# Spimp/sparc_ldpc

Measured on AMD Instinct MI355X. Metric: decoded codewords/sec (T AMP iters) at L=512,M=512; achieved HBM GB/s vs roofline, higher is better.
Workload: dtype f32; 1 GPU; BASELINE configs[1]: L=512 M=512 R=1 P=4, T=64, single codeword; L=512, M=512, n=4608, T=64, backend=hadamard, precision=fp32, early_stop=False, parallelism=reps sharded over 1 GPU(s)

## Files before the change

### include/sparc_amp.h

```cpp
#ifndef SPARC_AMP_H
#define SPARC_AMP_H

#include <stdint.h>

#ifdef __cplusplus
extern "C" {
#endif

typedef struct sa_ctx sa_ctx;

enum {
  SA_OK = 0,
  SA_ERR_ARG = -1,
  SA_ERR_HIP = -2,
  SA_ERR_NOMEM = -3,
  SA_ERR_ORDERING = -4,
  SA_ERR_UNSUPPORTED = -5,
  SA_ERR_NO_DEVICE = -6
};

enum {
  SA_BACKEND_HADAMARD = 0,
  SA_BACKEND_DENSE = 1,
  SA_BACKEND_HOST = 2,
// ... 17 lines not shown
  SA_PLAN_NO_SEC3 = 1 << 1,
  SA_PLAN_ROW16 = 1 << 2,
  SA_PLAN_NO_ROW16 = 1 << 3,
  SA_PLAN_NO_PT = 1 << 4,
  SA_PLAN_ZIL = 1 << 5,
  SA_PLAN_NO_ZIL = 1 << 6,
  SA_PLAN_WB8 = 1 << 7,
  SA_PLAN_WB16 = 1 << 8,
  SA_PLAN_NO_BANKS = 1 << 9,
  SA_PLAN_EAGER = 1 << 10,
  SA_PLAN_ONE_PASS = 1 << 11,
  SA_PLAN_NO_LANES = 1 << 12,
  SA_PLAN_SEC4Q = 1 << 13,
  SA_PLAN_NO_SEC4Q = 1 << 14,
  SA_PLAN_NO_FUSED_TAIL = 1 << 15,
  SA_PLAN_ALL = (1 << 16) - 1
};
int sa_create_ex(sa_ctx** out, int L, int M, int n, const uint32_t* ordering,
                 int backend, int precision, int device, int plan);

int sa_create_matrix(sa_ctx** out, int L, int M, int n, const double* A,
                     int precision, int device);

int sa_create_matrix_random(sa_ctx** out, int L, int M, int n, uint64_t seed, double scale,
                            int precision, int device);

int sa_subset(const sa_ctx* parent, const int64_t* sections, int Ls, sa_ctx** out);

int sa_create_twin(sa_ctx* src, sa_ctx** out);

void sa_destroy(sa_ctx* ctx);
// ... 108 lines not shown
```

### sparc_ldpc_amd/_lib.py

```python
from __future__ import annotations

import ctypes as ct
import os

import numpy as np

LIB_NAME = "libsparc_amp.so"
LIB_PATH = os.environ.get("SPARC_AMP_LIB") or os.path.join(os.path.dirname(os.path.abspath(__file__)), LIB_NAME)

SA_OK = 0
SA_ERR_ARG = -1
SA_ERR_HIP = -2
SA_ERR_NOMEM = -3
SA_ERR_ORDERING = -4
SA_ERR_UNSUPPORTED = -5
SA_ERR_NO_DEVICE = -6

SA_BACKEND_HADAMARD = 0
SA_BACKEND_DENSE = 1
SA_BACKEND_HOST = 2
SA_BACKEND_MATRIX = 3
SA_PREC_F32 = 0
SA_PREC_F64 = 1
SA_FLAG_NO_EARLY_STOP = 1
SA_FLAG_BETA0 = 0x100
SA_PTR_DEVICE = 0x200
SA_SE_MAX_M = 4096
SA_LLR_MODES = {"reference": 0, "two_sided": 1}

SA_PLAN = {
    "SEC3": 1 << 0, "NO_SEC3": 1 << 1, "ROW16": 1 << 2, "NO_ROW16": 1 << 3, "NO_PT": 1 << 4,
    "ZIL": 1 << 5, "NO_ZIL": 1 << 6, "WB8": 1 << 7, "WB16": 1 << 8, "NO_BANKS": 1 << 9, "EAGER": 1 << 10,
    "ONE_PASS": 1 << 11, "NO_LANES": 1 << 12, "SEC4Q": 1 << 13, "NO_SEC4Q": 1 << 14,
    "NO_FUSED_TAIL": 1 << 15,
}


def plan_bits(plan) -> int:
    if plan is None:
        return 0
    if isinstance(plan, int):
        return plan
    if isinstance(plan, str):
        plan = [plan]
    bits = 0
    for name in plan:
        key = name.upper()
        if key not in SA_PLAN:
            raise ValueError(f"unknown plan option {name!r}; known: {sorted(SA_PLAN)}")
# ... 142 lines not shown
```

### sparc_ldpc_amd/csrc/sa_common.h

```cpp
#pragma once
#include <hip/hip_runtime.h>
#include <hip/hip_ext.h>

#include <cfloat>
#include <cmath>
#include <cstdint>
#include <cstdio>
#include <cstdlib>
#include <cstring>
#include <algorithm>
#include <map>
#include <random>
#include <thread>
#include <string>
#include <tuple>
#include <type_traits>
#include <vector>

#include "sparc_amp.h"
#include "sa_shape.h"

namespace sa {

extern thread_local std::string g_err;
// ... 702 lines not shown
enum { SEC_AMP = 0, SEC_AZ = 1, SEC_AB = 2 };
enum { ROW_INIT0 = 0, ROW_INIT = 1, ROW_AMP = 2, ROW_ABOUT = 3 };


template <typename real>
struct SecArgs {
  const uint16_t* __restrict__ inv;
  const uint16_t* __restrict__ invb;
  const uint16_t* __restrict__ invl;
  const uint32_t* __restrict__ hs;
  const ushort4* __restrict__ fwd;
  const ushort4* __restrict__ fwdb;
  const uint32_t* __restrict__ fwd2;
  const uint32_t* __restrict__ fwd3;
  const uint32_t* __restrict__ inv32;
  const real* __restrict__ c;
  const real* __restrict__ z;
  real* __restrict__ beta;
  real* __restrict__ beta_out;
  real* __restrict__ out;
  real* __restrict__ abp;
  real* __restrict__ bbp;
  const real* __restrict__ zzp;
  real* __restrict__ tau;
  int* __restrict__ iters;
  int L, M, n, w, nhi, G, NZ, T1, t, mode, early_stop;
  int cst;
  int RS;
  int pt;
  int B, NC;
  int zil;
  int gpx;
  real sqrt_n;
  const int* tb;
  int dead;
  int bzero;
  int32_t* dec;
  int itset;
};

template <typename real>
struct RowArgs {
  const real* __restrict__ tau;
  const real* __restrict__ y;
  const real* __restrict__ z_in;
  const real* __restrict__ bbp;
  const real* __restrict__ Pb;
  const real* __restrict__ abp;
  int n, G, Gb, NZ, T1, t, mode, early_stop;
  int Pbst;
  int pt;
  int Bc;
  int itset;
// ... 91 lines not shown
      int e0 = elem_index<E>(lane, i);
      e0 = e0 < M ? e0 : 0;
      const unsigned bo = (off0 + (unsigned)(h * M + e0)) * 2u;
      if constexpr (Q == 4) {
        tb[hh][i / Q] = ld_off(reinterpret_cast<const ushort4*>(base), bo);
      } else if constexpr (Q == 2) {
        const ushort2 t2 = ld_off(reinterpret_cast<const ushort2*>(base), bo);
        tb[hh][i / Q] = make_ushort4(t2.x, t2.y, 0, 0);
      } else {
        tb[hh][i / Q] = make_ushort4(ld_off(base, bo), 0, 0, 0);
      }
    }
  }
}

template <typename real, int E, int KH>
__device__ __forceinline__ void gather_buckets(const real* zs, int h0, int nhi,
                                               const ushort4 (&tb)[KH][(E + 3) / 4], real (&v)[E]) {
  constexpr int Q = E < 4 ? E : 4;
  if constexpr (KH * E <= 64) {
    if (h0 + KH <= nhi) {
      real zz[KH][E];
#pragma unroll
      for (int hh = 0; hh < KH; ++hh)
#pragma unroll
        for (int i = 0; i < E; i += Q) {
          const ushort4 r4 = tb[hh][i / Q];
          const unsigned short rr[4] = {r4.x, r4.y, r4.z, r4.w};
#pragma unroll
          for (int q = 0; q < Q; ++q) {
// ... 92 lines not shown
```

### sparc_ldpc_amd/csrc/sa_host.h

```cpp
#pragma once
#include "sa_common.h"
#include "sa_tables.h"

namespace sa {

struct Prof {
  std::vector<std::tuple<int, hipEvent_t, hipEvent_t>> ev;
  int rep = 1;
  bool dispatch = false;
  int kind = 0;
  int begin(hipStream_t s, int k) {
    kind = k;
    if (dispatch) return 0;
    hipEvent_t a = nullptr, b = nullptr;
    if (add(&a, &b)) return -1;
    return hipEventRecord(a, s) == hipSuccess ? 0 : -1;
  }
  void end(hipStream_t s) {
    if (!dispatch) (void)hipEventRecord(std::get<2>(ev.back()), s);
  }
  int add(hipEvent_t* a, hipEvent_t* b) {
    *a = *b = nullptr;
    if (hipEventCreate(a) != hipSuccess || hipEventCreate(b) != hipSuccess) return -1;
    ev.emplace_back(kind, *a, *b);
// ... 144 lines not shown
  a.abp = (real*)ln.d_abp; a.bbp = (real*)ln.d_bbp; a.zzp = (const real*)ln.d_zzp;
  a.tau = (real*)ln.d_tau; a.iters = ln.d_iters;
  a.L = c->L; a.M = c->M; a.n = c->n; a.w = c->w; a.nhi = c->nhi; a.G = c->G; a.NZ = p.nz;
  a.T1 = c->Tcap + 1; a.t = t; a.mode = mode; a.early_stop = early_stop;
  a.RS = 1;
  a.pt = 0;
  a.B = 0; a.NC = 0; a.zil = 0; a.gpx = 1 << 20;
  a.cst = c->pb_on ? c->L : 0;
  if (c->pb_on) a.c = (const real*)c->d_cb;
  a.sqrt_n = (real)std::sqrt((double)c->n);
  a.tb = tb;
  a.dead = c->dead;
  a.bzero = 0;
  a.dec = nullptr;
  a.itset = 0;
  return a;
}

template <typename real>
RowArgs<real> row_args(sa_ctx* c, const Plan& p, int mode, int t, int early_stop, int G, int Gb, const int* tb = nullptr) {
  RowArgs<real> a;
  const sa_lane& ln = c->at();
  a.y = (const real*)ln.d_y; a.z = (real*)ln.d_z; a.z_in = a.z; a.abp = (const real*)ln.d_abp;
  a.bbp = (const real*)ln.d_bbp; a.zzp = (real*)ln.d_zzp; a.tau = (const real*)ln.d_tau;
  a.out = (real*)c->d_out;
  a.n = c->n; a.G = G; a.NZ = p.nz;
  a.Gb = Gb; a.T1 = c->Tcap + 1; a.t = t; a.mode = mode;
  a.early_stop = early_stop;
  a.sqrt_n = c->backend != SA_BACKEND_HADAMARD ? (real)1 : (real)std::sqrt((double)c->n);
  a.Pb = c->pb_on ? (const real*)c->d_Pb : (const real*)c->d_P1;
// ... 105 lines not shown
```

### sparc_ldpc_amd/csrc/sa_host_check.cpp

```cpp
#include <algorithm>
#include <cstdio>
#include <cstdlib>
#include <cstring>
#include <numeric>

#include "sa_shape.h"
#include "sa_tables.h"

using namespace sa;

static int usage() {
  std::fprintf(stderr, "usage: sa_host_check shape L M n backend prec plan n_cus B\n"
                       "       sa_host_check sweep L M backend prec plan n_cus B n0 n1\n"
                       "       sa_host_check tables L M n prec plan\n");
  return 2;
}

static int shape_of(Shape& s, int L, int M, int n, int backend, int prec, int plan, int n_cus) {
  std::string err;
  int rc = SA_OK;
  if (L <= 0 || M <= 0 || n <= 0 || n_cus <= 0 || backend < SA_BACKEND_HADAMARD || backend > SA_BACKEND_MATRIX ||
      (prec != SA_PREC_F32 && prec != SA_PREC_F64) || (plan & ~SA_PLAN_ALL)) {
    rc = SA_ERR_ARG;
    err = "bad arguments";
  }
  if (!rc) rc = shape_limits(M, n, backend, err);
  if (!rc) rc = shape_for(s, L, M, n, backend, prec, plan, n_cus, err);
  if (rc) std::printf("{\"error\": %d, \"message\": \"%s\"}\n", rc, err.c_str());
  return rc;
// ... 212 lines not shown
  std::vector<uint16_t> inv, fwd;
  std::vector<uint32_t> inv32;
  if (s.big ? check_inv(s, ord, inv32) : check_inv(s, ord, inv)) return 1;
  if (check_fwd(s, ord, fwd)) return 1;
  const bool secb = s.CB > 0 && !s.big, banked = invb_banked(s);
  if (secb && check_fwdb(s, fwd)) return 1;
  if (banked && check_banked(s, inv)) return 1;
  std::printf("{\"ok\": 1, \"M\": %d, \"dead\": %d, \"w\": %d, \"E\": %d, \"big\": %d, \"sec3\": %d, \"CB\": %d, \"WB\": %d, "
              "\"fwdb\": %d, \"fwdb_lanes\": %d, \"banked\": %d, \"kh\": %d, \"search\": %d}\n",
              s.M, s.dead, s.w, s.E, s.big ? 1 : 0, s.sec3 ? 1 : 0, s.CB, s.WB, secb ? 1 : 0,
              secb ? (s.CB * (int)rsz(&s) == 16 ? 16 : 32) : 0, banked ? 1 : 0, banked ? invb_kh(s) : 0,
              (plan & SA_PLAN_NO_BANKS) ? 0 : 1);
  return 0;
}

int main(int argc, char** argv) {
  if (argc < 2) return usage();
  std::vector<int> a;
  for (int i = 2; i < argc; ++i) a.push_back(std::atoi(argv[i]));
  if (!std::strcmp(argv[1], "shape") && a.size() == 8) return cmd_shape(a[0], a[1], a[2], a[3], a[4], a[5], a[6], a[7]);
  if (!std::strcmp(argv[1], "sweep") && a.size() == 9)
    return cmd_sweep(a[0], a[1], a[2], a[3], a[4], a[5], a[6], a[7], a[8]);
  if (!std::strcmp(argv[1], "tables") && a.size() == 5) return cmd_tables(a[0], a[1], a[2], a[3], a[4]);
  return usage();
}
```

### sparc_ldpc_amd/csrc/sa_sec.hip

```cpp
#include "sa_host.h"

namespace sa {



template <typename real, int E>
__global__ void __launch_bounds__(256) k_sec(SecArgs<real> a) {
  STAMP(0);
  extern __shared__ __attribute__((aligned(16))) unsigned char smem[];
  constexpr int KH = E >= 16 ? 2 : (E >= 8 ? 16 : 16);
  constexpr int NQ = (E + 3) / 4;
  constexpr int KR = 8;
  int g, rsi;
  if (a.RS > 1 && (a.G & 7) == 0) {
    const int j = blockIdx.x, u = j >> 3;
    rsi = u % a.RS;
    g = (u / a.RS) * 8 + (j & 7);
  } else {
    g = blockIdx.x / a.RS;
    rsi = blockIdx.x % a.RS;
  }
  const int b = blockIdx.y;
  const int rows_per = (a.n + a.RS - 1) / a.RS;
  const int rb0 = rsi * rows_per, rb1 = min(a.n, rb0 + rows_per);
// ... 466 lines not shown
template <typename real, int QW, bool MAX>
__device__ __forceinline__ real combine_q(const real* red, int w0, int f) {
  real x[QW];
#pragma unroll
  for (int j = 0; j < QW; ++j) x[j] = red[(w0 + j) * 4 + f];
#pragma unroll
  for (int span = 1; span < QW; span <<= 1)
#pragma unroll
    for (int j = 0; j < QW; j += 2 * span) {
      if constexpr (MAX) x[j] = x[j] > x[j + span] ? x[j] : x[j + span];
      else x[j] = x[j] + x[j + span];
    }
  return x[0];
}

template <typename real, int EQ, int QW, int SPW = 2>
__device__ __forceinline__ void secq_body(const SecArgs<real>& a) {
  static_assert(SPW == 2 || SPW == 3 || SPW == 4, "sections per workgroup");
  STAMP(0);
  extern __shared__ __attribute__((aligned(16))) unsigned char smem[];
  constexpr int NT = SPW * QW * 64;
  constexpr int KH = EQ >= 8 ? 4 : ((SPW == 3 || (SPW == 4 && sizeof(real) == 8)) ? 8 : 16);
  constexpr int NQ = (EQ + 3) / 4;
  constexpr int KR = ((SPW == 3 ? 8448 : 4608) + NT - 1) / NT;
  constexpr int FW = SPW == 4 ? 2 : 1;
  const int g = blockIdx.x, b = blockIdx.y;
  const int tid = threadIdx.x, lane = tid & 63, wv = tid >> 6;
  const int sidx = wv / QW, q = wv % QW;
  const int M = a.M, n = a.n, Mq = M / QW;
  const size_t LM = (size_t)a.L * M;
  const int l = g * SPW + sidx;
  const bool have = l < a.L;
  const int lc = have ? l : a.L - 1;
// ... 3 lines not shown
  const int zslots = ((n + 1) * (int)sizeof(real) + 15) / 16 * 16 / (int)sizeof(real);
  real* ts = zs + zslots;
  real* xb = ts + SPW * M;
  real* red = xb + SPW * M;

  real v[EQ];
  real bprev[EQ];
  const real* bl = a.beta + (size_t)b * LM + (size_t)lc * M + eoff;
  real* blo = a.beta_out + (size_t)b * LM + (size_t)lc * M + eoff;
  const uint16_t* ibase = a.inv + (size_t)g * SPW * a.w;
  const unsigned ioff = (unsigned)((lc - g * SPW) * a.w + eoff);
  const uint32_t* fw = (SPW == 3 ? a.fwd3 : a.fwd2) + (size_t)(SPW == 4 ? 2 * g : g) * n;
  const uint32_t* fw1 = a.fwd2 + (size_t)(2 * g + 1 < (a.L + 1) / 2 ? 2 * g + 1 : 2 * g) * n;
  ushort4 tb[KH][NQ];
  uint32_t f[KR][FW];

  const real* zb = a.z + (size_t)b * n;
  ZStage<real, NT> zst;
  const real* zzb = a.zzp + (size_t)b * a.NZ;
  ZZParts<real, 5> zz;
  const bool dma = stage_z_dma<real, NT>(zb, zs, n, tid);
  if (!dma) zst.issue(zb, n, tid);
  zz.issue(zzb, a.NZ, lane);
  const real last = a.t > 0 ? ld_vmem(a.tau + (size_t)b * a.T1 + a.t - 1) : (real)0;
  load_buckets_off<EQ, KH>(ibase, ioff, 0, a.nhi, M, lane, tb);
  load_section<real, EQ>(bl, bprev, lane, Mq);
  const real cl = ld_vmem(a.c + (size_t)b * a.cst + lc);
  const real tau = zz.tau(zzb, a.NZ, n);
  if (a.bzero) {
#pragma unroll
    for (int i = 0; i < EQ; ++i) bprev[i] = 0;
  }
  const bool stop = a.early_stop && (tau == last);
  if (g == 0 && tid == 0) {
    a.tau[(size_t)b * a.T1 + a.t] = tau;
    if (stop && a.iters[b] < 0) a.iters[b] = a.t;
    if (a.itset != 0 && !stop) a.iters[b] = a.itset;
  }
  if (stop) {
    if (dma) asm volatile("s_waitcnt vmcnt(0)" ::: "memory");
    if (a.bzero && have) {
      store_section<real, EQ>(a.beta + (size_t)b * LM + (size_t)lc * M + eoff, bprev, lane, Mq);
// ... 3 lines not shown
  const real tau2 = tau * tau;
  const real inv_sn = (real)1 / a.sqrt_n;
  const real kk = cl / tau2;
  STAMP(1);
  if (!dma) zst.store(zs, zb, n, tid);
  else finish_z_dma<real>(zb, zs, n, tid);
  __syncthreads();
  STAMP(2);
#ifdef SA_STAMPS
  asm volatile("s_waitcnt vmcnt(0)" ::: "memory");
  STAMP(10);
#endif
#pragma unroll
  for (int i = 0; i < EQ; ++i) v[i] = 0;
  for (int h0 = 0; h0 < a.nhi; h0 += KH) {
    ushort4 tn[KH][NQ];
    const bool more = h0 + KH < a.nhi;
    if (more) load_buckets_off<EQ, KH>(ibase, ioff, h0 + KH, a.nhi, M, lane, tn);
    gather_buckets<real, EQ, KH>(zs, h0, a.nhi, tb, v);
    if (more) {
#pragma unroll
      for (int hh = 0; hh < KH; ++hh)
#pragma unroll
        for (int j = 0; j < NQ; ++j) tb[hh][j] = tn[hh][j];
    }
  }
  real* xs = xb + sidx * M;
#pragma unroll
  for (int u = 0; u < KR; ++u) {
    const int r = u * NT + tid;
    f[u][0] = ld_off(fw, (unsigned)(r < n ? r : 0) * 4u);
    if constexpr (SPW == 4) f[u][1] = ld_off(fw1, (unsigned)(r < n ? r : 0) * 4u);
  }
  STAMP(3);
  fwht_wave<real, EQ>(v, lane, 64);
  topq_stage<real, EQ, QW>(v, xs, lane, q);
  STAMP(4);


  real mx = neg_inf<real>();
#pragma unroll
  for (int i = 0; i < EQ; ++i) {
    v[i] = fma(v[i], inv_sn, bprev[i]) * kk;
    mx = v[i] > mx ? v[i] : mx;
  }
  mx = wave_max(mx);
  if (lane == 0) red[wv * 4] = mx;
// ... 32 lines not shown
    for (int m = 32; m >= 1; m >>= 1) {
      const real ob = __shfl_xor(dbest, m);
      const int oi = __shfl_xor(dbi, m);
      if (ob > dbest || (ob == dbest && oi < dbi)) { dbest = ob; dbi = oi; }
    }
  }

  STAMP(5);
  fwht_wave<real, EQ>(v, lane, 64);
  topq_stage<real, EQ, QW>(v, xs, lane, q);
  STAMP(6);
  {
    real* tl = ts + sidx * M + eoff;
#pragma unroll
    for (int i = 0; i < EQ; ++i) tl[elem_index<EQ>(lane, i)] = v[i];
  }
  if (lane == 0) {
    red[wv * 4 + 3] = bb;
    if (a.dec) {
      red[wv * 4] = dbest;
      red[wv * 4 + 1] = (real)dbi;
    }
  }
  __syncthreads();
  STAMP(7);
  if (a.dec && have && q == 0 && lane == 0) {
    real best = red[wv * 4];
    int bi = (int)red[wv * 4 + 1];
#pragma unroll
    for (int j = 1; j < QW; ++j) {
// ... 9 lines not shown
    if constexpr (SPW == 4) bsum += red[3 * QW * 4 + 3];
    a.bbp[(size_t)b * a.G + g] = bsum;
  }
  real* abp = a.abp + ((size_t)b * a.G + g) * n;
  const int psh = a.pt == 16 ? 4 : 5;
  const size_t npad = (size_t)((n + (1 << psh) - 1) >> psh) << psh;
  real* abq = a.abp + (size_t)b * a.G * npad + ((size_t)g << psh);
  real* const sbase = a.pt ? abq : abp;
  const int sh = a.pt ? psh : 31;
  const size_t gstride = (size_t)a.G << sh;
  const int smask = (int)((1u << sh) - 1u);
  static_assert(NT % 32 == 0, "a pass of rows is a whole number of row blocks");
  const size_t ustep = sh < 31 ? (size_t)(NT >> sh) * gstride : (size_t)NT;
  for (int r0 = 0; r0 < n; r0 += NT * KR) {
    if (r0 > 0) {
#pragma unroll
      for (int u = 0; u < KR; ++u) {
        const int r = r0 + u * NT + tid;
        f[u][0] = fw[r < n ? r : 0];
        if constexpr (SPW == 4) f[u][1] = fw1[r < n ? r : 0];
      }
    }
    real* const pbase = sbase + (size_t)((r0 + tid) >> sh) * gstride + ((r0 + tid) & smask);
    auto row = [&](int u, int r) {
      real t;
      if constexpr (SPW == 2) {
        const uint32_t e = f[u][0];
        const real v0 = ts[e & 0x7fffu];
        const real v1 = ts[M + ((e >> 16) & 0x7fffu)];
        t = (e & 0x8000u) ? -v0 : v0;
        t += (e & 0x80000000u) ? -v1 : v1;
      } else if constexpr (SPW == 4) {
        const uint32_t e = f[u][0], e1 = f[u][1];
        const real v0 = ts[e & 0x7fffu];
        const real v1 = ts[M + ((e >> 16) & 0x7fffu)];
        const real v2 = ts[2 * M + (e1 & 0x7fffu)];
        const real v3 = ts[3 * M + ((e1 >> 16) & 0x7fffu)];
        t = (e & 0x8000u) ? -v0 : v0;
        t += (e & 0x80000000u) ? -v1 : v1;
        real t1 = (e1 & 0x8000u) ? -v2 : v2;
        t1 += (e1 & 0x80000000u) ? -v3 : v3;
// ... 21 lines not shown
#pragma unroll
      for (int u = 0; u < KR; ++u) {
        const int r = r0 + u * NT + tid;
        if (r < n) row(u, r);
      }
    }
  }
#ifdef SA_STAMPS
  STAMP(8);
  asm volatile("s_waitcnt vmcnt(0)" ::: "memory");
  STAMP(9);
#endif
}

template <typename real, int E4>
__global__ void __launch_bounds__(512) k_sec4(SecArgs<real> a) { secq_body<real, E4, 4, 2>(a); }
template <typename real, int E4>
__global__ void __launch_bounds__(768) k_sec43(SecArgs<real> a) { secq_body<real, E4, 4, 3>(a); }
template <typename real, int E4>
__global__ void __launch_bounds__(1024) k_sec44(SecArgs<real> a) { secq_body<real, E4, 4, 4>(a); }

template <typename real, int E>
void launch_sec_e(sa_ctx* c, const Plan& p, int B, SecArgs<real> a) {
  a.RS = p.rs;
  dim3 grid(c->G * a.RS, B);
  if (c->prof) c->prof->begin(c->at().stream, K_SEC);
  if (c->big)
    plaunch(c, k_secg<real, E>, grid, 256, c->sec_lds, a);
  else
    plaunch(c, k_sec<real, E>, grid, 256, c->sec_lds, a);
  if (c->prof) c->prof->end(c->at().stream);
}

template <typename real>
int launch_sec2(sa_ctx* c, const Plan& p, int B, int t, int es, void* bin, void* bout, int bzero, int32_t* dec,
                int itset) {
  SecArgs<real> a = sec_args<real>(c, p, SEC_AMP, t, es);
  a.pt = p.pt;
  if (bzero && !p.bzero()) return fail(SA_ERR_UNSUPPORTED, "k_sec2 reads its previous estimate");
  if ((dec || itset) && (!p.bzero() || es || c->dead))
    return fail(SA_ERR_UNSUPPORTED, "launch_sec2: no fused decision on this path");
  a.bzero = bzero;
  a.dec = dec;
  a.itset = itset;
  a.beta = (real*)bin;
  a.beta_out = (real*)bout;
  a.G = p.G;
  dim3 grid(a.G, B);
  if (c->prof) c->prof->begin(c->at().stream, K_SEC);
  switch (p.sec) {
    case SA_SEC_K_SEC43:
      switch (c->M / 256) {
        case 1: plaunch(c, k_sec43<real, 1>, grid, 768, c->sec3_lds, a); break;
        case 2: plaunch(c, k_sec43<real, 2>, grid, 768, c->sec3_lds, a); break;
        default: return fail(SA_ERR_UNSUPPORTED, "k_sec43: M");
      }
      break;
    case SA_SEC_K_SEC44:
      switch (c->M / 256) {
        case 1: plaunch(c, k_sec44<real, 1>, grid, 1024, c->sec4q_lds, a); break;
        case 2: plaunch(c, k_sec44<real, 2>, grid, 1024, c->sec4q_lds, a); break;
        default: return fail(SA_ERR_UNSUPPORTED, "k_sec44: M");
// ... 89 lines not shown
```

### sparc_ldpc_amd/csrc/sa_shape.h

```cpp
#pragma once
#include <algorithm>
#include <cstddef>
#include <string>

#include "sparc_amp.h"

namespace sa {

constexpr int kSpw = 4;
constexpr int kRowsPerBlk = 64;
constexpr int kRow2Rows = 32;
constexpr int kSG = 16;
constexpr size_t kSecbL2 = (size_t)5 << 19;
constexpr int kWB = 8, kWB16 = 16;
constexpr int kInvbZeroRows = 16;
constexpr int kSecbKH32 = 2, kSecbKH64 = 2;
constexpr size_t kLdsBytes = 160 * 1024;

inline int ilog2(int x) {
  int r = 0;
  while ((1 << r) < x) ++r;
  return r;
}

struct Shape {
  int L = 0, n = 0, backend = 0, prec = 0;
  int plan = 0;
  int n_cus = 256;
  int M = 0, Mu = 0, dead = 0;
  bool pow2 = true;
  int w = 0, nhi = 0, E = 1;
  bool big = false;
  int NZ = 0, NZ16 = 0, NZh = 0, NZ4 = 0, NZ2 = 0;
  bool row16 = false;
  bool pt_on = false;
  int G = 0;
  size_t sec_lds = 0;
  int G2 = 0;
  size_t sec2_lds = 0;
  bool sec4 = false;
  size_t sec4_lds = 0;
  int G3 = 0;
  bool sec3 = false;
  size_t sec3_lds = 0;
  int G4 = 0;
  bool sec4q = false;
  size_t sec4q_lds = 0;
  int WB = 8;
  int CB = 0;
  int Gb = 0;
  int gpx = 1 << 20;
  size_t secb_lds = 0;
  int Gd = 0;
};

inline size_t rsz(const Shape* s) { return s->prec == SA_PREC_F64 ? 8 : 4; }

inline size_t zbytes(int n, size_t s) { return ((size_t)(n + 1) * s + 15) / 16 * 16; }
inline size_t sec_lds_need(int M, int n, size_t s, bool z) {
  return (z ? zbytes(n, s) : 0) + (size_t)kSpw * M * s + (size_t)kSpw * s;
}
inline size_t sec2_need(int M, int n, size_t s) {
// ... 99 lines not shown
    const bool over = c.G2 > c.n_cus || (s == 8 && c.G2 == c.n_cus);
    const bool want = (plan & SA_PLAN_SEC3) ? true : (plan & SA_PLAN_NO_SEC3) ? false : (over && G3 <= c.n_cus);
    if (fits && want) {
      c.sec3 = true;
      c.G3 = G3;
      c.sec3_lds = sec43_need(M, n, s);
    }
    const bool fits4q = c.sec4 && backend == SA_BACKEND_HADAMARD && M <= 512 && sec44_need(M, n, s) <= kLdsBytes;
    if (fits4q && (plan & SA_PLAN_SEC4Q) && !(plan & (SA_PLAN_SEC3 | SA_PLAN_NO_SEC4Q))) {
      c.sec4q = true;
      c.sec3 = false;
      c.G4 = (L + 3) / 4;
      c.sec4q_lds = sec44_need(M, n, s);
    }
    if (c.G2 == c.n_cus && !(plan & (SA_PLAN_ROW16 | SA_PLAN_NO_SEC3))) c.row16 = false;
  }
  return SA_OK;
}

constexpr int kI8MinB = 4;
constexpr int kI8MaxS = 16;
constexpr int kFMinB = 4;
constexpr int kFMaxS = 16;

inline bool is_dense(const Shape& c) { return c.backend == SA_BACKEND_DENSE || c.backend == SA_BACKEND_MATRIX; }
inline bool use_i8(const Shape& c, int B) { return c.backend == SA_BACKEND_DENSE && B >= kI8MinB; }
inline bool use_fgemm(const Shape& c, int B) { return c.backend == SA_BACKEND_MATRIX && B >= kFMinB; }
inline bool use_batched(const Shape& c, int B) { return c.CB > 0 && B >= 4; }

inline bool zil_for(const Shape& c, int B) {
// ... 78 lines not shown
```

### sparc_ldpc_amd/csrc/sa_tables.h

```cpp
#pragma once
#include <cstdint>
#include <random>
#include <vector>

#include "sa_shape.h"

namespace sa {

struct Tables {
  uint16_t* inv = nullptr;
  uint32_t* inv32 = nullptr;
  uint16_t* invb = nullptr;
  uint16_t* invl = nullptr;
  uint32_t* hs = nullptr;
  uint16_t* fwd = nullptr;
  uint16_t* fwdb = nullptr;
  uint32_t* fwd2 = nullptr;
  uint32_t* fwd3 = nullptr;
  bool invb_done = false;
};

inline uint16_t fwd_entry(uint32_t v, int lgM, int M) {
  return (uint16_t)((v & (uint32_t)(M - 1)) | ((__builtin_popcount(v >> lgM) & 1u) << 15));
}

inline int fwd_groups(int L) { return (L + kSG - 1) / kSG * (kSG / kSpw); }

template <typename T>
bool inv_row(const uint32_t* o, int l, int n, int w, T* il, std::string& bad) {
  for (int r = 0; r < n; ++r) {
    const uint32_t v = o[r];
    if (v == 0 || v >= (uint32_t)w) {
      bad = "ordering[" + std::to_string(l) + "," + std::to_string(r) + "] = " + std::to_string(v) +
// ... 6 lines not shown
    }
    il[v] = (T)r;
  }
  return true;
}

inline void fwd_section(const uint32_t* o, int l, int n, int M, uint16_t* fwd, uint32_t* fwd2, uint32_t* fwd3) {
  const int lgM = ilog2(M);
  for (int r = 0; r < n; ++r) {
    const uint16_t e = fwd_entry(o[r], lgM, M);
    fwd[((size_t)(l / kSpw) * n + r) * kSpw + (l % kSpw)] = e;
    if (fwd2) fwd2[(size_t)(l / 2) * n + r] |= (uint32_t)e << (16 * (l & 1));
    if (fwd3)
      fwd3[(size_t)(l / 3) * n + r] |= (uint32_t)((e & 0x1ffu) | ((e >> 15) << 9)) << (10 * (l % 3));
  }
}

constexpr int kLdsGroups16[4][16] = {
    {0, 1, 2, 3, 12, 13, 14, 15, 20, 21, 22, 23, 24, 25, 26, 27},
    {4, 5, 6, 7, 8, 9, 10, 11, 16, 17, 18, 19, 28, 29, 30, 31},
    {32, 33, 34, 35, 44, 45, 46, 47, 52, 53, 54, 55, 56, 57, 58, 59},
    {36, 37, 38, 39, 40, 41, 42, 43, 48, 49, 50, 51, 60, 61, 62, 63}};

inline bool secb_rows16(const Shape& c) {
  return c.backend == SA_BACKEND_HADAMARD && c.CB > 0 && c.CB * (int)rsz(&c) == 16 && !c.big;
}
inline bool invb_banked(const Shape& c) {
  return secb_rows16(c) && !(c.plan & SA_PLAN_NO_BANKS) && c.E >= 4 && c.nhi >= 2 && c.n + kInvbZeroRows <= 65535;
}
inline int invb_kh(const Shape& c) { return c.prec == SA_PREC_F32 ? kSecbKH32 : kSecbKH64; }
// ... 196 lines not shown
```

### sparc_ldpc_amd/csrc/sa_tables.hip

```cpp

#include "sa_host.h"

namespace sa {

void tables_free(Tables& t) {
  void* all[] = {t.inv, t.inv32, t.invb, t.invl, t.hs, t.fwd, t.fwdb, t.fwd2, t.fwd3};
  for (void* p : all) dev_free(p);
  t = Tables();
}

template <typename T>
static int table_upload(sa_ctx* c, T** dst, const std::vector<T>& src) {
  if (int rc = dev_alloc(c, (void**)dst, src.size() * sizeof(T))) return rc;
  HIP_TRY(hipMemcpyAsync(*dst, src.data(), src.size() * sizeof(T), hipMemcpyHostToDevice, c->at().stream));
  return SA_OK;
}

template <typename T>
static int fill_inv(const sa_ctx* c, std::vector<T>& inv) {
  const int L = c->L, n = c->n, w = c->w;
  inv.assign((size_t)L * w, (T)n);
  std::vector<std::string> bad((size_t)L);
  parallel_for(L, 1, [&](int l) {
    inv_row(c->ordering.data() + (size_t)l * n, l, n, w, inv.data() + (size_t)l * w, bad[l]);
// ... 26 lines not shown
static void host_drop(sa_ctx* c) {
  std::vector<uint16_t>().swap(c->h_inv);
  std::vector<uint16_t>().swap(c->h_fwd);
}

int build_tables(sa_ctx* c) {
  Tables& t = c->tab;
  std::vector<uint32_t> inv32, fwd2, fwd3;
  int rc = c->big ? fill_inv(c, inv32) : fill_inv(c, c->h_inv);
  if (rc) return rc;
  fill_fwd(c, c->h_fwd, c->big ? nullptr : &fwd2, c->sec3 ? &fwd3 : nullptr);
  rc = c->big ? table_upload(c, &t.inv32, inv32) : table_upload(c, &t.inv, c->h_inv);
  if (!rc) rc = table_upload(c, &t.fwd, c->h_fwd);
  if (!rc && !c->big) rc = table_upload(c, &t.fwd2, fwd2);
  if (!rc && c->sec3) rc = table_upload(c, &t.fwd3, fwd3);
  HIP_TRY(hipStreamSynchronize(c->at().stream));
  if (rc) return rc;
  if (!(c->backend == SA_BACKEND_HADAMARD && c->CB > 0)) host_drop(c);
  return SA_OK;
}

static int build_banked(sa_ctx* c) {
  const int L = c->L, w = c->w;
  const std::vector<int> sets = invb_sets(c->E, c->prec == SA_PREC_F32);
  const uint16_t* inv = host_inv(c).data();
  std::vector<uint16_t> out((size_t)L * w, 0);
  std::vector<uint32_t> hs((size_t)L, 0);
  parallel_for(L, 1, [&](int l) {
    banked_section(c->M, c->n, c->nhi, l, inv + (size_t)l * w, out.data() + (size_t)l * w, sets, 16, 16, hs.data(),
                   invb_kh(*c));
// ... 60 lines not shown
```

Measured before the change: 2371 codewords/s.

## Bit-pack inverse bucket and forward pair tables to cut table traffic

```diff
diff --git a/include/sparc_amp.h b/include/sparc_amp.h
--- a/include/sparc_amp.h
+++ b/include/sparc_amp.h
@@ -55,7 +55,8 @@
   SA_PLAN_SEC4Q = 1 << 13,
   SA_PLAN_NO_SEC4Q = 1 << 14,
   SA_PLAN_NO_FUSED_TAIL = 1 << 15,
-  SA_PLAN_ALL = (1 << 16) - 1
+  SA_PLAN_NO_PACK = 1 << 16,
+  SA_PLAN_ALL = (1 << 17) - 1
 };
 int sa_create_ex(sa_ctx** out, int L, int M, int n, const uint32_t* ordering,
                  int backend, int precision, int device, int plan);
diff --git a/sparc_ldpc_amd/_lib.py b/sparc_ldpc_amd/_lib.py
--- a/sparc_ldpc_amd/_lib.py
+++ b/sparc_ldpc_amd/_lib.py
@@ -32,7 +32,7 @@
     "SEC3": 1 << 0, "NO_SEC3": 1 << 1, "ROW16": 1 << 2, "NO_ROW16": 1 << 3, "NO_PT": 1 << 4,
     "ZIL": 1 << 5, "NO_ZIL": 1 << 6, "WB8": 1 << 7, "WB16": 1 << 8, "NO_BANKS": 1 << 9, "EAGER": 1 << 10,
     "ONE_PASS": 1 << 11, "NO_LANES": 1 << 12, "SEC4Q": 1 << 13, "NO_SEC4Q": 1 << 14,
-    "NO_FUSED_TAIL": 1 << 15,
+    "NO_FUSED_TAIL": 1 << 15, "NO_PACK": 1 << 16,
 }
 
 
diff --git a/sparc_ldpc_amd/csrc/sa_common.h b/sparc_ldpc_amd/csrc/sa_common.h
--- a/sparc_ldpc_amd/csrc/sa_common.h
+++ b/sparc_ldpc_amd/csrc/sa_common.h
@@ -740,6 +740,8 @@
   const uint32_t* __restrict__ fwd2;
   const uint32_t* __restrict__ fwd3;
   const uint32_t* __restrict__ inv32;
+  const uint32_t* __restrict__ invp;
+  const uint64_t* __restrict__ fwd2p;
   const real* __restrict__ c;
   const real* __restrict__ z;
   real* __restrict__ beta;
@@ -763,6 +765,7 @@
   int bzero;
   int32_t* dec;
   int itset;
+  int pj;
 };
 
 template <typename real>
@@ -884,6 +887,46 @@
   }
 }
 
+using u4v = unsigned __attribute__((ext_vector_type(4)));
+
+template <int E, int KH>
+__device__ __forceinline__ void load_packed(const uint32_t* __restrict__ base, unsigned woff, int blk, int lane,
+                                            uint32_t (&pw)[pack_rd(E, KH)]) {
+  constexpr int RD = pack_rd(E, KH), NV = RD / 4;
+  const unsigned b0 = woff + (unsigned)blk * (64u * RD * 4u);
+#pragma unroll
+  for (int v = 0; v < NV; ++v) {
+    const u4v t = ld_off(reinterpret_cast<const u4v*>(base), b0 + (unsigned)(v * 256 + lane * 4) * 4u);
+    pw[4 * v] = t.x; pw[4 * v + 1] = t.y; pw[4 * v + 2] = t.z; pw[4 * v + 3] = t.w;
+  }
+#pragma unroll
+  for (int j = 4 * NV; j < RD; ++j) pw[j] = ld_off(base, b0 + (unsigned)(NV * 256 + (j - 4 * NV) * 64 + lane) * 4u);
+}
+
+template <int E, int KH>
+__device__ __forceinline__ void unpack_pairs(const uint32_t (&pw)[pack_rd(E, KH)], uint32_t (&tw)[KH]) {
+  static_assert(E <= 2, "packed records: one dword per step");
+#pragma unroll
+  for (int hh = 0; hh < KH; ++hh) {
+    uint32_t w = 0;
+#pragma unroll
+    for (int i = 0; i < E; ++i) {
+      const int bit = (hh * E + i) * kPackBits, dw = bit / 32, sh = bit % 32;
+      uint32_t x = pw[dw] >> sh;
+      if (sh + kPackBits > 32) x |= pw[dw + 1] << (32 - sh);
+      w |= (x & ((1u << kPackBits) - 1u)) << (16 * i);
+    }
+    asm("" : "+v"(w));
+    tw[hh] = w;
+  }
+}
+template <int KH>
+__device__ __forceinline__ void pairs_to_buckets(const uint32_t (&tw)[KH], ushort4 (&tb)[KH][1]) {
+#pragma unroll
+  for (int hh = 0; hh < KH; ++hh)
+    tb[hh][0] = make_ushort4((unsigned short)(tw[hh] & 0xffffu), (unsigned short)(tw[hh] >> 16), 0, 0);
+}
+
 template <typename real, int E, int KH>
 __device__ __forceinline__ void gather_buckets(const real* zs, int h0, int nhi,
                                                const ushort4 (&tb)[KH][(E + 3) / 4], real (&v)[E]) {
diff --git a/sparc_ldpc_amd/csrc/sa_host.h b/sparc_ldpc_amd/csrc/sa_host.h
--- a/sparc_ldpc_amd/csrc/sa_host.h
+++ b/sparc_ldpc_amd/csrc/sa_host.h
@@ -182,6 +182,7 @@
   a.bzero = 0;
   a.dec = nullptr;
   a.itset = 0;
+  a.invp = nullptr; a.fwd2p = nullptr; a.pj = 0;
   return a;
 }
 
diff --git a/sparc_ldpc_amd/csrc/sa_host_check.cpp b/sparc_ldpc_amd/csrc/sa_host_check.cpp
--- a/sparc_ldpc_amd/csrc/sa_host_check.cpp
+++ b/sparc_ldpc_amd/csrc/sa_host_check.cpp
@@ -12,7 +12,8 @@
 static int usage() {
   std::fprintf(stderr, "usage: sa_host_check shape L M n backend prec plan n_cus B\n"
                        "       sa_host_check sweep L M backend prec plan n_cus B n0 n1\n"
-                       "       sa_host_check tables L M n prec plan\n");
+                       "       sa_host_check tables L M n prec plan\n"
+                       "       sa_host_check packed L M n prec plan\n");
   return 2;
 }
 
@@ -255,6 +256,75 @@
   return 0;
 }
 
+static int cmd_packed(int L, int M, int n, int prec, int plan) {
+  Shape s;
+  if (shape_of(s, L, M, n, SA_BACKEND_HADAMARD, prec, plan, Shape().n_cus)) return 1;
+  size_t invp_bytes = 0, fwd2p_bytes = 0;
+  if (s.pack_inv || s.pack_fwd) {
+    std::vector<uint32_t> ord((size_t)L * n), all(s.w - 1);
+    for (int l = 0; l < L; ++l) {
+      std::mt19937 rng(0x0d0000u + (uint32_t)l);
+      std::iota(all.begin(), all.end(), 1u);
+      std::shuffle(all.begin(), all.end(), rng);
+      std::copy(all.begin(), all.begin() + n, ord.begin() + (size_t)l * n);
+    }
+    std::vector<uint16_t> inv((size_t)L * s.w, (uint16_t)n), fwd((size_t)fwd_groups(L) * n * kSpw, 0);
+    std::vector<uint32_t> fwd2((size_t)s.G2 * n, 0);
+    for (int l = 0; l < L; ++l) {
+      std::string bad;
+      CHECK(inv_row(ord.data() + (size_t)l * n, l, n, s.w, inv.data() + (size_t)l * s.w, bad), "inv_row: %s", bad.c_str());
+      fwd_section(ord.data() + (size_t)l * n, l, n, s.M, fwd.data(), fwd2.data(), nullptr);
+    }
+    if (s.pack_inv) {
+      const int kh = s.pack_kh, EQ = s.M / 256, rd = pack_rd(EQ, kh);
+      CHECK(EQ >= 1 && EQ <= 2 && n <= kPackMaxN, "packed bucket records at M = %d, n = %d", s.M, n);
+      const size_t per = pack_inv_section_dwords(s.M, s.nhi, kh);
+      CHECK(per == (size_t)4 * ((s.nhi + kh - 1) / kh) * 64 * rd, "section size");
+      std::vector<int> seen((size_t)64 * rd, 0);
+      for (int lane = 0; lane < 64; ++lane)
+        for (int j = 0; j < rd; ++j) {
+          const unsigned pos = pack_dword_pos(rd, lane, j);
+          CHECK(pos < (unsigned)(64 * rd) && !seen[pos]++, "pack_dword_pos(%d, %d, %d) = %u", rd, lane, j, pos);
+        }
+      std::vector<uint32_t> invp((size_t)L * per, 0);
+      for (int l = 0; l < L; ++l) pack_inv_section(s.M, n, s.nhi, kh, inv.data() + (size_t)l * s.w, invp.data() + (size_t)l * per);
+      for (int l = 0; l < L; ++l)
+        for (int h = 0; h < s.nhi; ++h)
+          for (int col = 0; col < s.M; ++col) {
+            const uint32_t got = pack_inv_get(s.M, s.nhi, kh, invp.data() + (size_t)l * per, h, col);
+            CHECK(got == inv[(size_t)l * s.w + (size_t)h * s.M + col], "invp[%d] step %d column %d = %u, inv has %u", l, h, col,
+                  got, (unsigned)inv[(size_t)l * s.w + (size_t)h * s.M + col]);
+          }
+      for (int l = 0; l < L; ++l)
+        for (int h = s.nhi; h < (s.nhi + kh - 1) / kh * kh; ++h)
+          for (int col = 0; col < s.M; ++col)
+            CHECK(pack_inv_get(s.M, s.nhi, kh, invp.data() + (size_t)l * per, h, col) == (uint32_t)n,
+                  "invp[%d] step %d (past nhi) column %d is not the zero slot", l, h, col);
+      invp_bytes = invp.size() * 4;
+    }
+    if (s.pack_fwd) {
+      CHECK(s.M <= 512 && !s.sec4q, "packed pair table at M = %d, quads %d", s.M, s.sec4q ? 1 : 0);
+      const int words = pack_fwd_words(n);
+      const size_t per = (size_t)words * kPackNT;
+      std::vector<uint64_t> fwd2p((size_t)s.G2 * per, 0);
+      for (int g = 0; g < s.G2; ++g) pack_fwd_pair(n, fwd2.data() + (size_t)g * n, fwd2p.data() + (size_t)g * per);
+      for (int g = 0; g < s.G2; ++g)
+        for (int r = 0; r < words * 3 * kPackNT; ++r) {
+          const uint32_t want = fwd2[(size_t)g * n + (r < n ? r : 0)], got = pack_fwd_get(fwd2p.data() + (size_t)g * per, r);
+          CHECK(got == want, "fwd2p[%d] row %d = %#x, fwd2 has %#x", g, r, got, want);
+        }
+      for (uint64_t wv : fwd2p) CHECK((wv >> 60) == 0, "fwd2p: bits past the three fields");
+      fwd2p_bytes = fwd2p.size() * 8;
+    }
+  }
+  std::printf("{\"ok\": 1, \"M\": %d, \"n\": %d, \"nhi\": %d, \"pack_inv\": %d, \"pack_fwd\": %d, \"kh\": %d, \"rd\": %d, "
+              "\"blocks\": %d, \"words\": %d, \"inv_bytes\": %zu, \"invp_bytes\": %zu, \"fwd2_bytes\": %zu, \"fwd2p_bytes\": %zu}\n",
+              s.M, n, s.nhi, s.pack_inv ? 1 : 0, s.pack_fwd ? 1 : 0, s.pack_kh,
+              s.pack_inv ? pack_rd(s.M / 256, s.pack_kh) : 0, s.pack_inv ? (s.nhi + s.pack_kh - 1) / s.pack_kh : 0,
+              s.pack_fwd ? pack_fwd_words(n) : 0, (size_t)L * s.w * 2, invp_bytes, (size_t)s.G2 * n * 4, fwd2p_bytes);
+  return 0;
+}
+
 int main(int argc, char** argv) {
   if (argc < 2) return usage();
   std::vector<int> a;
@@ -263,5 +333,6 @@
   if (!std::strcmp(argv[1], "sweep") && a.size() == 9)
     return cmd_sweep(a[0], a[1], a[2], a[3], a[4], a[5], a[6], a[7], a[8]);
   if (!std::strcmp(argv[1], "tables") && a.size() == 5) return cmd_tables(a[0], a[1], a[2], a[3], a[4]);
+  if (!std::strcmp(argv[1], "packed") && a.size() == 5) return cmd_packed(a[0], a[1], a[2], a[3], a[4]);
   return usage();
 }
diff --git a/sparc_ldpc_amd/csrc/sa_sec.hip b/sparc_ldpc_amd/csrc/sa_sec.hip
--- a/sparc_ldpc_amd/csrc/sa_sec.hip
+++ b/sparc_ldpc_amd/csrc/sa_sec.hip
@@ -504,9 +504,11 @@
   return x[0];
 }
 
-template <typename real, int EQ, int QW, int SPW = 2>
+template <typename real, int EQ, int QW, int SPW = 2, bool PKI = false, bool PKF = false>
 __device__ __forceinline__ void secq_body(const SecArgs<real>& a) {
   static_assert(SPW == 2 || SPW == 3 || SPW == 4, "sections per workgroup");
+  static_assert(!PKI || (EQ <= 2 && QW == 4 && SPW != 3), "packed bucket records: pairs and quads, M <= 512");
+  static_assert(!PKF || (EQ <= 2 && QW == 4 && SPW == 2), "packed pair table: pairs, M <= 512");
   STAMP(0);
   extern __shared__ __attribute__((aligned(16))) unsigned char smem[];
   constexpr int NT = SPW * QW * 64;
@@ -540,6 +542,14 @@
   const uint32_t* fw1 = a.fwd2 + (size_t)(2 * g + 1 < (a.L + 1) / 2 ? 2 * g + 1 : 2 * g) * n;
   ushort4 tb[KH][NQ];
   uint32_t f[KR][FW];
+  constexpr int RD = pack_rd(EQ <= 2 ? EQ : 1, KH);
+  static_assert(!PKF || (NT == kPackNT && KR == kPackKR), "the packed pair table's thread and row counts");
+  const int pnb = (a.nhi + KH - 1) / KH;
+  const uint32_t* pkbase = a.invp + (size_t)g * SPW * 4 * pnb * (64 * RD);
+  const unsigned pkoff = (unsigned)(((lc - g * SPW) * 4 + q) * pnb) * (64u * RD * 4u);
+  const uint64_t* fwp = a.fwd2p + (size_t)g * a.pj * NT;
+  uint32_t pw[RD];
+  uint64_t fq[KR / 3 + 1];
 
   const real* zb = a.z + (size_t)b * n;
   ZStage<real, NT> zst;
@@ -549,9 +559,12 @@
   if (!dma) zst.issue(zb, n, tid);
   zz.issue(zzb, a.NZ, lane);
   const real last = a.t > 0 ? ld_vmem(a.tau + (size_t)b * a.T1 + a.t - 1) : (real)0;
-  load_buckets_off<EQ, KH>(ibase, ioff, 0, a.nhi, M, lane, tb);
+  if constexpr (PKI) load_packed<EQ, KH>(pkbase, pkoff, 0, lane, pw);
+  else load_buckets_off<EQ, KH>(ibase, ioff, 0, a.nhi, M, lane, tb);
   load_section<real, EQ>(bl, bprev, lane, Mq);
   const real cl = ld_vmem(a.c + (size_t)b * a.cst + lc);
+  uint32_t tw[KH];
+  if constexpr (PKI) unpack_pairs<EQ, KH>(pw, tw);
   const real tau = zz.tau(zzb, a.NZ, n);
   if (a.bzero) {
 #pragma unroll
@@ -585,23 +598,36 @@
 #pragma unroll
   for (int i = 0; i < EQ; ++i) v[i] = 0;
   for (int h0 = 0; h0 < a.nhi; h0 += KH) {
-    ushort4 tn[KH][NQ];
     const bool more = h0 + KH < a.nhi;
-    if (more) load_buckets_off<EQ, KH>(ibase, ioff, h0 + KH, a.nhi, M, lane, tn);
-    gather_buckets<real, EQ, KH>(zs, h0, a.nhi, tb, v);
-    if (more) {
-#pragma unroll
-      for (int hh = 0; hh < KH; ++hh)
-#pragma unroll
-        for (int j = 0; j < NQ; ++j) tb[hh][j] = tn[hh][j];
+    if constexpr (PKI) {
+      uint32_t pn[RD];
+      if (more) load_packed<EQ, KH>(pkbase, pkoff, h0 / KH + 1, lane, pn);
+      pairs_to_buckets<KH>(tw, tb);
+      gather_buckets<real, EQ, KH>(zs, h0, a.nhi, tb, v);
+      if (more) unpack_pairs<EQ, KH>(pn, tw);
+    } else {
+      ushort4 tn[KH][NQ];
+      if (more) load_buckets_off<EQ, KH>(ibase, ioff, h0 + KH, a.nhi, M, lane, tn);
+      gather_buckets<real, EQ, KH>(zs, h0, a.nhi, tb, v);
+      if (more) {
+#pragma unroll
+        for (int hh = 0; hh < KH; ++hh)
+#pragma unroll
+          for (int j = 0; j < NQ; ++j) tb[hh][j] = tn[hh][j];
+      }
     }
   }
   real* xs = xb + sidx * M;
-#pragma unroll
-  for (int u = 0; u < KR; ++u) {
-    const int r = u * NT + tid;
-    f[u][0] = ld_off(fw, (unsigned)(r < n ? r : 0) * 4u);
-    if constexpr (SPW == 4) f[u][1] = ld_off(fw1, (unsigned)(r < n ? r : 0) * 4u);
+  if constexpr (PKF) {
+#pragma unroll
+    for (int j = 0; j < KR / 3; ++j) fq[j] = ld_off(fwp, (unsigned)(j * NT + tid) * 8u);
+  } else {
+#pragma unroll
+    for (int u = 0; u < KR; ++u) {
+      const int r = u * NT + tid;
+      f[u][0] = ld_off(fw, (unsigned)(r < n ? r : 0) * 4u);
+      if constexpr (SPW == 4) f[u][1] = ld_off(fw1, (unsigned)(r < n ? r : 0) * 4u);
+    }
   }
   STAMP(3);
   fwht_wave<real, EQ>(v, lane, 64);
@@ -664,6 +690,14 @@
     real* tl = ts + sidx * M + eoff;
 #pragma unroll
     for (int i = 0; i < EQ; ++i) tl[elem_index<EQ>(lane, i)] = v[i];
+  }
+  if constexpr (PKF) {
+#pragma unroll
+    for (int u = 0; u < KR; ++u) {
+      uint32_t e = (uint32_t)(fq[u / 3] >> (20 * (u % 3))) & 0xfffffu;
+      asm("" : "+v"(e));
+      f[u][0] = e;
+    }
   }
   if (lane == 0) {
     red[wv * 4 + 3] = bb;
@@ -703,17 +737,34 @@
   const size_t ustep = sh < 31 ? (size_t)(NT >> sh) * gstride : (size_t)NT;
   for (int r0 = 0; r0 < n; r0 += NT * KR) {
     if (r0 > 0) {
-#pragma unroll
-      for (int u = 0; u < KR; ++u) {
-        const int r = r0 + u * NT + tid;
-        f[u][0] = fw[r < n ? r : 0];
-        if constexpr (SPW == 4) f[u][1] = fw1[r < n ? r : 0];
+      if constexpr (PKF) {
+#pragma unroll
+        for (int j = 0; j < KR / 3; ++j) fq[j] = fwp[(size_t)(r0 / (NT * KR) * (KR / 3) + j) * NT + tid];
+#pragma unroll
+        for (int u = 0; u < KR; ++u) {
+          uint32_t e = (uint32_t)(fq[u / 3] >> (20 * (u % 3))) & 0xfffffu;
+          asm("" : "+v"(e));
+          f[u][0] = e;
+        }
+      } else {
+#pragma unroll
+        for (int u = 0; u < KR; ++u) {
+          const int r = r0 + u * NT + tid;
+          f[u][0] = fw[r < n ? r : 0];
+          if constexpr (SPW == 4) f[u][1] = fw1[r < n ? r : 0];
+        }
       }
     }
     real* const pbase = sbase + (size_t)((r0 + tid) >> sh) * gstride + ((r0 + tid) & smask);
     auto row = [&](int u, int r) {
       real t;
-      if constexpr (SPW == 2) {
+      if constexpr (PKF) {
+        const uint32_t e = f[u][0];
+        const real v0 = ts[e & 0x1ffu];
+        const real v1 = ts[M + ((e >> 10) & 0x1ffu)];
+        t = (e & 0x200u) ? -v0 : v0;
+        t += (e & 0x80000u) ? -v1 : v1;
+      } else if constexpr (SPW == 2) {
         const uint32_t e = f[u][0];
         const real v0 = ts[e & 0x7fffu];
         const real v1 = ts[M + ((e >> 16) & 0x7fffu)];
@@ -765,11 +816,20 @@
 }
 
 template <typename real, int E4>
-__global__ void __launch_bounds__(512) k_sec4(SecArgs<real> a) { secq_body<real, E4, 4, 2>(a); }
+__global__ void __launch_bounds__(512) k_sec4(SecArgs<real> a) {
+  if constexpr (E4 <= 2) {
+    if (__builtin_expect(!(a.invp && a.fwd2p), 0)) return secq_body<real, E4, 4, 2>(a);
+    return secq_body<real, E4, 4, 2, true, true>(a);
+  }
+  secq_body<real, E4, 4, 2>(a);
+}
 template <typename real, int E4>
 __global__ void __launch_bounds__(768) k_sec43(SecArgs<real> a) { secq_body<real, E4, 4, 3>(a); }
 template <typename real, int E4>
-__global__ void __launch_bounds__(1024) k_sec44(SecArgs<real> a) { secq_body<real, E4, 4, 4>(a); }
+__global__ void __launch_bounds__(1024) k_sec44(SecArgs<real> a) {
+  if (__builtin_expect(!a.invp, 0)) return secq_body<real, E4, 4, 4>(a);
+  secq_body<real, E4, 4, 4, true>(a);
+}
 
 template <typename real, int E>
 void launch_sec_e(sa_ctx* c, const Plan& p, int B, SecArgs<real> a) {
@@ -797,6 +857,13 @@
   a.beta = (real*)bin;
   a.beta_out = (real*)bout;
   a.G = p.G;
+  if (p.sec == SA_SEC_K_SEC4 || p.sec == SA_SEC_K_SEC44) {
+    if (c->pack_inv) a.invp = c->tab.invp;
+    if (c->pack_fwd && p.sec == SA_SEC_K_SEC4) {
+      a.fwd2p = c->tab.fwd2p;
+      a.pj = pack_fwd_words(c->n);
+    }
+  }
   dim3 grid(a.G, B);
   if (c->prof) c->prof->begin(c->at().stream, K_SEC);
   switch (p.sec) {
diff --git a/sparc_ldpc_amd/csrc/sa_shape.h b/sparc_ldpc_amd/csrc/sa_shape.h
--- a/sparc_ldpc_amd/csrc/sa_shape.h
+++ b/sparc_ldpc_amd/csrc/sa_shape.h
@@ -16,6 +16,16 @@
 constexpr int kInvbZeroRows = 16;
 constexpr int kSecbKH32 = 2, kSecbKH64 = 2;
 constexpr size_t kLdsBytes = 160 * 1024;
+
+constexpr int kPackBits = 13;
+constexpr int kPackMaxN = (1 << kPackBits) - 2;
+constexpr int pack_rd(int EQ, int KH) { return (EQ * KH * kPackBits + 31) / 32; }
+constexpr unsigned pack_dword_pos(int rd, int lane, int j) {
+  return j < rd / 4 * 4 ? (unsigned)((j / 4) * 256 + lane * 4 + j % 4)
+                        : (unsigned)(rd / 4 * 256 + (j - rd / 4 * 4) * 64 + lane);
+}
+constexpr int kPackNT = 512, kPackKR = 9, kPackRows = kPackNT * kPackKR;
+constexpr int pack_fwd_words(int n) { return (n + kPackRows - 1) / kPackRows * (kPackKR / 3); }
 
 inline int ilog2(int x) {
   int r = 0;
@@ -46,6 +56,9 @@
   int G4 = 0;
   bool sec4q = false;
   size_t sec4q_lds = 0;
+  bool pack_inv = false;
+  bool pack_fwd = false;
+  int pack_kh = 0;
   int WB = 8;
   int CB = 0;
   int Gb = 0;
@@ -175,6 +188,10 @@
       c.sec4q_lds = sec44_need(M, n, s);
     }
     if (c.G2 == c.n_cus && !(plan & (SA_PLAN_ROW16 | SA_PLAN_NO_SEC3))) c.row16 = false;
+    const bool packable = c.sec4 && !c.sec3 && backend == SA_BACKEND_HADAMARD && M <= 512 && n <= kPackMaxN;
+    c.pack_inv = packable && !(plan & SA_PLAN_NO_PACK);
+    c.pack_fwd = packable && !c.sec4q && !(plan & SA_PLAN_NO_PACK);
+    c.pack_kh = c.sec4q && s == 8 ? 8 : 16;
   }
   return SA_OK;
 }
diff --git a/sparc_ldpc_amd/csrc/sa_tables.h b/sparc_ldpc_amd/csrc/sa_tables.h
--- a/sparc_ldpc_amd/csrc/sa_tables.h
+++ b/sparc_ldpc_amd/csrc/sa_tables.h
@@ -17,6 +17,8 @@
   uint16_t* fwdb = nullptr;
   uint32_t* fwd2 = nullptr;
   uint32_t* fwd3 = nullptr;
+  uint32_t* invp = nullptr;
+  uint64_t* fwd2p = nullptr;
   bool invb_done = false;
 };
 
@@ -53,6 +55,70 @@
     if (fwd3)
       fwd3[(size_t)(l / 3) * n + r] |= (uint32_t)((e & 0x1ffu) | ((e >> 15) << 9)) << (10 * (l % 3));
   }
+}
+
+inline int elem_index_host(int E, int lane, int i) {
+  const int Q = E < 4 ? E : 4;
+  return (i / Q) * (64 * Q) + lane * Q + (i % Q);
+}
+inline size_t pack_inv_section_dwords(int M, int nhi, int kh) {
+  return (size_t)4 * ((nhi + kh - 1) / kh) * 64 * pack_rd(M / 256, kh);
+}
+inline void pack_entry_at(int EQ, int hh, int i, int& dw, int& sh) {
+  const int bit = (hh * EQ + i) * kPackBits;
+  dw = bit / 32;
+  sh = bit % 32;
+}
+inline void pack_inv_section(int M, int n, int nhi, int kh, const uint16_t* inv_l, uint32_t* out) {
+  const int EQ = M / 256, Mq = M / 4, rd = pack_rd(EQ, kh), nb = (nhi + kh - 1) / kh;
+  for (int q = 0; q < 4; ++q)
+    for (int blk = 0; blk < nb; ++blk) {
+      uint32_t* wb = out + ((size_t)q * nb + blk) * 64 * rd;
+      for (int lane = 0; lane < 64; ++lane)
+        for (int hh = 0; hh < kh; ++hh)
+          for (int i = 0; i < EQ; ++i) {
+            const int h = blk * kh + hh;
+            const uint32_t v = h < nhi ? inv_l[(size_t)h * M + q * Mq + elem_index_host(EQ, lane, i)] : (uint32_t)n;
+            int dw, sh;
+            pack_entry_at(EQ, hh, i, dw, sh);
+            wb[pack_dword_pos(rd, lane, dw)] |= v << sh;
+            if (sh + kPackBits > 32) wb[pack_dword_pos(rd, lane, dw + 1)] |= v >> (32 - sh);
+          }
+    }
+}
+inline uint32_t pack_inv_get(int M, int nhi, int kh, const uint32_t* sec, int h, int col) {
+  const int EQ = M / 256, Mq = M / 4, rd = pack_rd(EQ, kh), nb = (nhi + kh - 1) / kh;
+  const int q = col / Mq, e = col % Mq, Q = EQ < 4 ? EQ : 4;
+  const int lane = (e % (64 * Q)) / Q, i = (e / (64 * Q)) * Q + e % Q;
+  const uint32_t* wb = sec + ((size_t)q * nb + h / kh) * 64 * rd;
+  int dw, sh;
+  pack_entry_at(EQ, h % kh, i, dw, sh);
+  uint64_t x = wb[pack_dword_pos(rd, lane, dw)];
+  if (sh + kPackBits > 32) x |= (uint64_t)wb[pack_dword_pos(rd, lane, dw + 1)] << 32;
+  return (uint32_t)(x >> sh) & ((1u << kPackBits) - 1u);
+}
+
+inline uint32_t pack_fwd_field(uint32_t e) {
+  return (e & 0x1ffu) | (((e >> 15) & 1u) << 9) | (((e >> 16) & 0x1ffu) << 10) | ((e >> 31) << 19);
+}
+inline uint32_t pack_fwd_entry(uint32_t f) {
+  return (f & 0x1ffu) | (((f >> 9) & 1u) << 15) | (((f >> 10) & 0x1ffu) << 16) | (((f >> 19) & 1u) << 31);
+}
+inline void pack_fwd_pair(int n, const uint32_t* fwd2_g, uint64_t* out) {
+  const int words = pack_fwd_words(n);
+  for (int j = 0; j < words; ++j)
+    for (int tid = 0; tid < kPackNT; ++tid) {
+      uint64_t wv = 0;
+      for (int f = 0; f < 3; ++f) {
+        const int r = (3 * j + f) * kPackNT + tid;
+        wv |= (uint64_t)pack_fwd_field(fwd2_g[r < n ? r : 0]) << (20 * f);
+      }
+      out[(size_t)j * kPackNT + tid] = wv;
+    }
+}
+inline uint32_t pack_fwd_get(const uint64_t* pair, int r) {
+  const int u = r / kPackNT, tid = r % kPackNT;
+  return pack_fwd_entry((uint32_t)(pair[(size_t)(u / 3) * kPackNT + tid] >> (20 * (u % 3))) & 0xfffffu);
 }
 
 constexpr int kLdsGroups16[4][16] = {
diff --git a/sparc_ldpc_amd/csrc/sa_tables.hip b/sparc_ldpc_amd/csrc/sa_tables.hip
--- a/sparc_ldpc_amd/csrc/sa_tables.hip
+++ b/sparc_ldpc_amd/csrc/sa_tables.hip
@@ -4,7 +4,7 @@
 namespace sa {
 
 void tables_free(Tables& t) {
-  void* all[] = {t.inv, t.inv32, t.invb, t.invl, t.hs, t.fwd, t.fwdb, t.fwd2, t.fwd3};
+  void* all[] = {t.inv, t.inv32, t.invb, t.invl, t.hs, t.fwd, t.fwdb, t.fwd2, t.fwd3, t.invp, t.fwd2p};
   for (void* p : all) dev_free(p);
   t = Tables();
 }
@@ -64,6 +64,24 @@
   if (!rc) rc = table_upload(c, &t.fwd, c->h_fwd);
   if (!rc && !c->big) rc = table_upload(c, &t.fwd2, fwd2);
   if (!rc && c->sec3) rc = table_upload(c, &t.fwd3, fwd3);
+  std::vector<uint32_t> invp;
+  std::vector<uint64_t> fwd2p;
+  if (!rc && c->pack_inv) {
+    const size_t per = pack_inv_section_dwords(c->M, c->nhi, c->pack_kh);
+    invp.assign((size_t)c->L * per, 0);
+    parallel_for(c->L, 1, [&](int l) {
+      pack_inv_section(c->M, c->n, c->nhi, c->pack_kh, c->h_inv.data() + (size_t)l * c->w, invp.data() + (size_t)l * per);
+    });
+    rc = table_upload(c, &t.invp, invp);
+  }
+  if (!rc && c->pack_fwd) {
+    const size_t per = (size_t)pack_fwd_words(c->n) * kPackNT;
+    fwd2p.assign((size_t)c->G2 * per, 0);
+    parallel_for(c->G2, 1, [&](int g) {
+      pack_fwd_pair(c->n, fwd2.data() + (size_t)g * c->n, fwd2p.data() + (size_t)g * per);
+    });
+    rc = table_upload(c, &t.fwd2p, fwd2p);
+  }
   HIP_TRY(hipStreamSynchronize(c->at().stream));
   if (rc) return rc;
   if (!(c->backend == SA_BACKEND_HADAMARD && c->CB > 0)) host_drop(c);
```

Result: faster. 2466 codewords/s, median of 6 (+4.0%).
